# pyannote/pyannote-audio

Hardware: NVIDIA H100
Metric: audio-hours/sec (RTF) community-1 diarization, 16kHz mono, 1/2/4/8 H100 (higher is better)
Workload: dtype f16 tensor-core trunk (f32 accumulate) + split-f16x3 tensor-core segmentation (f32-level accuracy) + f64 clustering

## Files before the change

pyannote_audio_b200/csrc/emb_conv.cu:

```cuda
#include "common.cuh"
#include "emb.cuh"
#include "tc_common.cuh"

namespace b200 {

constexpr int kWgThreads = 288;
constexpr int kTileM = 128;
constexpr int kRowHalo = 8;
constexpr int kMaxSlots = 16;

template <int N, bool WIDE = false, int MH = 1>
__device__ __forceinline__ void conv_epilogue(const float* acc, const ConvParams& p, size_t row, int w0) {
  const int lane = threadIdx.x & 31;
  const int c0 = 2 * (lane & 3) + (WIDE ? (int)blockIdx.y * N : 0);
#pragma unroll
  for (int m = 0; m < MH; ++m)
#pragma unroll
  for (int i = 0; i < 2; ++i) {
    const int w = w0 + 64 * m + ((threadIdx.x >> 5) & 3) * 16 + (lane >> 2) + 8 * i;
    if (w >= p.W_out) continue;
    const size_t pix = (row * p.W_out + w) * (size_t)(WIDE ? p.C_out : N);
    __half2 res[N / 8];
    if (N <= 128 && p.residual) {
#pragma unroll
      for (int j = 0; j < N / 8; ++j) res[j] = *reinterpret_cast<const __half2*>(p.residual + pix + 8 * j + c0);
    }
#pragma unroll
    for (int j = 0; j < N / 8; ++j) {
      const int c = 8 * j + c0;
      const float2 bb = __ldg(reinterpret_cast<const float2*>(p.bias + c));
      float a = acc[m * (N / 2) + 4 * j + 2 * i] + bb.x, d = acc[m * (N / 2) + 4 * j + 2 * i + 1] + bb.y;
      if (p.residual) {
        const float2 r = __half22float2(N <= 128 ? res[j] : *reinterpret_cast<const __half2*>(p.residual + pix + c));
        a += r.x;
        d += r.y;
      }
      if (p.relu) { a = fmaxf(a, 0.f); d = fmaxf(d, 0.f); }
      *reinterpret_cast<__half2*>(p.out + pix + c) = __floats2half2_rn(a, d);
    }
  }
}

template <int N, int CK, bool WIDE = false>
__global__ void __launch_bounds__(kWgThreads, N == 256 ? 1 : 2)
conv_tc_kernel(const __grid_constant__ CUtensorMap tmA, const __grid_constant__ CUtensorMap tmB, ConvParams p) {
  extern __shared__ uint8_t smem_raw[];
  const uint32_t raw = smem_u32(smem_raw);
  const uint32_t base = (raw + 1023u) & ~1023u;
  const uint32_t bar_full = base, bar_empty = base + 64;
  const uint32_t stage0 = base + 1024;
  const uint32_t stage_bytes = p.a_bytes + p.b_bytes;
  const int warp = threadIdx.x >> 5;
  const int wt = blockIdx.x % p.tiles_w;
  const int bh = blockIdx.x / p.tiles_w;
  const int cchunks = p.C_in / CK;

  if (threadIdx.x == 0) {
    for (uint32_t s = 0; s < p.nstages; ++s) { mbar_init(bar_full + 8 * s, 1); mbar_init(bar_empty + 8 * s, 2); }
    asm volatile("fence.mbarrier_init.release.cluster;" ::: "memory");
  }
  __syncthreads();

  if (warp == 8) {
    if ((threadIdx.x & 31) == 0) {
      prefetch_tensormap(&tmA);
      prefetch_tensormap(&tmB);
      const int h = bh % p.H_out, b = bh / p.H_out;
      const int w_base = wt * kTileM * p.stride - p.pad, h_base = h * p.stride - p.pad;
      uint32_t stage = 0, phase = 0;
      for (int kh = 0; kh < p.taps_h; ++kh)
        for (int kw = 0; kw < p.taps_w; ++kw)
          for (int cc = 0; cc < cchunks; ++cc) {
            mbar_wait(bar_empty + 8 * stage, phase ^ 1);
            mbar_expect_tx(bar_full + 8 * stage, p.a_tx + p.b_bytes);
            const uint32_t sa = stage0 + stage * stage_bytes;
            tma_load_4d(&tmA, bar_full + 8 * stage, sa, cc * CK, w_base + kw, h_base + kh, b);
            tma_load_3d(&tmB, bar_full + 8 * stage, sa + p.a_bytes, cc * CK, WIDE ? (int)blockIdx.y * N : 0,
                        kh * p.taps_w + kw);
            if (++stage == p.nstages) { stage = 0; phase ^= 1; }
          }
    }
    return;
  }

  const int wg = warp >> 2;
  constexpr uint32_t row_bytes = CK * 2;
  float acc[N / 2];
#pragma unroll
  for (int i = 0; i < N / 2; ++i) acc[i] = 0.f;
  const int kblocks = p.taps_h * p.taps_w * cchunks;
  uint32_t stage = 0, phase = 0, prev = 0;
  for (int kb = 0; kb < kblocks; ++kb) {
    mbar_wait(bar_full + 8 * stage, phase);
    const uint32_t st = stage0 + stage * stage_bytes;
    const uint32_t sa = st + (uint32_t)wg * 64u * row_bytes, sb = st + p.a_bytes;
    wg_fence();
    const uint64_t ad = wg_desc(sa, row_bytes), bd = wg_desc(sb, row_bytes);
#pragma unroll
    for (int k = 0; k < CK / 16; ++k) Wgmma<N>::mma(acc, ad + 2 * k, bd + 2 * k);
    wg_commit();
    wg_wait<1>();
    if (kb > 0 && (threadIdx.x & 127) == 0) mbar_arrive(bar_empty + 8 * prev);
    prev = stage;
    if (++stage == p.nstages) { stage = 0; phase ^= 1; }
  }
  wg_wait<0>();
  conv_epilogue<N, WIDE>(acc, p, (size_t)bh, wt * kTileM + wg * 64);
}

template <int N>
__device__ __forceinline__ void row_taps_c32(float (&acc)[2][N / 2], uint32_t sa, uint32_t wts) {
  constexpr uint32_t row_bytes = 64;
  const int warp = threadIdx.x >> 5, lane = threadIdx.x & 31;
#pragma unroll
  for (int kw = 0; kw < 3; ++kw) {
    uint32_t af[2][2][4];
#pragma unroll
    for (int m = 0; m < 2; ++m)
#pragma unroll
      for (int k = 0; k < 2; ++k) {
        const uint32_t row = (uint32_t)(m * 64 + (warp & 3) * 16 + (lane & 15) + kw);
        const uint32_t chunk = (uint32_t)(2 * k + (lane >> 4)) ^ ((row >> 1) & 3u);
        ldsm_x4(af[m][k], sa + row * row_bytes + chunk * 16u);
      }
    wg_fence();
    const uint64_t bd = wg_desc(wts + kw * N * row_bytes, row_bytes);
#pragma unroll
    for (int k = 0; k < 2; ++k)
#pragma unroll
      for (int m = 0; m < 2; ++m) WgmmaRS<N>::mma(acc[m], af[m][k], bd + 2 * k);
    wg_commit();
    wg_wait<0>();
  }
}

__device__ __forceinline__ void st_shared_u32(uint32_t a, uint32_t v) {
  asm volatile("st.shared.b32 [%0], %1;" ::"r"(a), "r"(v) : "memory");
}
__device__ __forceinline__ uint32_t ld_shared_u32(uint32_t a) {
  uint32_t v;
  asm volatile("ld.shared.b32 %0, [%1];" : "=r"(v) : "r"(a) : "memory");
  return v;
}
__device__ __forceinline__ uint32_t h2_bits(__half2 h) { return *reinterpret_cast<uint32_t*>(&h); }

template <int N>
struct RowPlan {
  static constexpr uint32_t kRowBytes = N * 2;
  static constexpr uint32_t kTapBytes = N * kRowBytes;
  static constexpr uint32_t kInTx = (kTileM + kRowHalo) * kRowBytes;
  static constexpr uint32_t kSlotBytes = (kInTx + 1023u) & ~1023u;
  static constexpr uint32_t kTileBytes = kTileM * kRowBytes;
  static constexpr uint32_t kSlots = N == 64 ? 7 : 8;
  static constexpr int kResLag = (int)kSlots - 2;
  static constexpr int kCtasPerSm = N == 32 ? 2 : 1;
  static constexpr size_t kBudget = N == 32 ? 113u * 1024 : 227u * 1024;
  static constexpr size_t kSmem = 2048 + 9 * kTapBytes + 2 * kTileBytes + kSlots * kSlotBytes;
  static_assert(N == 32 || N == 64, "row kernel: 32 or 64 channels");
  static_assert(kSlots >= 6 && kSlots <= kMaxSlots, "row ring: four slots in use and two ahead");
  static_assert(kSmem <= kBudget && kSmem + kSlotBytes > kBudget, "row plan: every slot that fits");
};

template <int N, int CK>
__global__ void __launch_bounds__(kWgThreads, N == 32 ? 2 : 1)
conv_row_kernel(const __grid_constant__ CUtensorMap tmA, const __grid_constant__ CUtensorMap tmB,
                const __grid_constant__ CUtensorMap tmR, const __grid_constant__ CUtensorMap tmO, ConvParams p) {
  using P = RowPlan<N>;
  static_assert(CK == N, "row kernel: one channel chunk");
  constexpr uint32_t row_bytes = P::kRowBytes;
  constexpr uint32_t b_tap_bytes = P::kTapBytes;
  constexpr uint32_t nslots = P::kSlots;
  extern __shared__ uint8_t smem_raw[];
  const uint32_t base = (smem_u32(smem_raw) + 1023u) & ~1023u;
  const uint32_t bar_w = base, bar_full = base + 8, bar_empty = base + 8 + 8 * kMaxSlots;
  const uint32_t tile_full = base + 512, tile_empty = base + 528;
  const uint32_t wts = base + 1024;
  const uint32_t tile0 = wts + 9 * b_tap_bytes;
  const uint32_t slot0 = tile0 + 2 * P::kTileBytes;
  const bool has_res = p.residual != nullptr;
  const int warp = threadIdx.x >> 5;

  if (threadIdx.x == 0) {
    mbar_init(bar_w, 1);
    for (uint32_t s = 0; s < nslots; ++s) { mbar_init(bar_full + 8 * s, 1); mbar_init(bar_empty + 8 * s, 3); }
    for (uint32_t s = 0; s < 2; ++s) { mbar_init(tile_full + 8 * s, 1); mbar_init(tile_empty + 8 * s, 1); }
    asm volatile("fence.mbarrier_init.release.cluster;" ::: "memory");
  }
  __syncthreads();

  if (warp == 8) {
    if ((threadIdx.x & 31) == 0) {
      prefetch_tensormap(&tmA);
      prefetch_tensormap(&tmB);
      if (has_res) prefetch_tensormap(&tmR);
      mbar_expect_tx(bar_w, 9 * b_tap_bytes);
      for (int kh = 0; kh < 3; ++kh) tma_load_3d(&tmB, bar_w, wts + 3 * kh * b_tap_bytes, 0, 0, 3 * kh);
      uint32_t s = 0;
      uint32_t k = 0;
      for (int u = blockIdx.x; u < p.num_tiles; u += gridDim.x) {
        const int wt = u % p.tiles_w, t = u / p.tiles_w;
        const int h0 = (t % p.bands) * p.band, b = t / p.bands;
        const int n = min(p.band, p.H_out - h0);
        auto stage_residual = [&](int j) {
          const uint32_t tile = k & 1, use = k >> 1;
          mbar_wait(tile_empty + 8 * tile, (use & 1) ^ 1);
          mbar_expect_tx(tile_full + 8 * tile, P::kTileBytes);
          tma_load_4d(&tmR, tile_full + 8 * tile, tile0 + tile * P::kTileBytes, 0, wt * kTileM, h0 + j, b);
          ++k;
        };
        for (int r = 0; r < n + 2; ++r, ++s) {
          const uint32_t slot = s % nslots;
          mbar_wait(bar_empty + 8 * slot, ((s / nslots) & 1) ^ 1);
          mbar_expect_tx(bar_full + 8 * slot, P::kInTx);
          tma_load_4d(&tmA, bar_full + 8 * slot, slot0 + slot * P::kSlotBytes, 0, wt * kTileM - 1, h0 - 1 + r, b);
          if (has_res && r >= P::kResLag) stage_residual(r - P::kResLag);
        }
        if (has_res)
          for (int j = max(0, n + 2 - P::kResLag); j < n; ++j) stage_residual(j);
      }
    }
    return;
  }

  const int wg = __shfl_sync(0xffffffffu, warp >> 2, 0);
  const int lane = threadIdx.x & 31;
  const bool leader = (threadIdx.x & 127) == 0;
  const uint32_t tile = tile0 + wg * P::kTileBytes;
  const int c0 = 2 * (lane & 3);
  float2 bias[N / 8];
#pragma unroll
  for (int j = 0; j < N / 8; ++j) bias[j] = __ldg(reinterpret_cast<const float2*>(p.bias + 8 * j + c0));
  if (leader) prefetch_tensormap(&tmO);
  mbar_wait(bar_w, 0);
  uint32_t s = 0;
  int item = 0;
  for (int u = blockIdx.x; u < p.num_tiles; u += gridDim.x) {
    const int wt = u % p.tiles_w, t = u / p.tiles_w;
    const int h0 = (t % p.bands) * p.band, b = t / p.bands;
    const int n = min(p.band, p.H_out - h0);
    for (int j = 0; j < n; ++j, ++item) {
      if ((item & 1) != wg) continue;
      float acc[2][N / 2];
#pragma unroll
      for (int m = 0; m < 2; ++m)
#pragma unroll
        for (int i = 0; i < N / 2; ++i) {
          acc[m][i] = 0.f;
          asm volatile("" : "+f"(acc[m][i]));
        }
#pragma unroll
      for (int kh = 0; kh < 3; ++kh) {
        const uint32_t q = s + j + kh, slot = q % nslots;
        mbar_wait(bar_full + 8 * slot, (q / nslots) & 1);
        const uint32_t sa = slot0 + slot * P::kSlotBytes;
        if constexpr (CK == 32) {
          row_taps_c32<N>(acc, sa, wts + 3 * kh * b_tap_bytes);
        } else {
          wg_fence();
#pragma unroll
          for (int kw = 0; kw < 3; ++kw) {
            const uint64_t bd = wg_desc(wts + (3 * kh + kw) * b_tap_bytes, row_bytes);
#pragma unroll
            for (int m = 0; m < 2; ++m) {
              const uint64_t ad = wg_desc(sa + (uint32_t)(m * 64 + kw) * row_bytes, row_bytes);
#pragma unroll
              for (int k = 0; k < CK / 16; ++k) Wgmma<N>::mma(acc[m], ad + 2 * k, bd + 2 * k);
            }
          }
          wg_commit();
        }
      }
      wg_wait<0>();
      if (leader)
#pragma unroll
        for (int kh = 0; kh < 3; ++kh)
          mbar_arrive_n(bar_empty + 8 * ((s + j + kh) % nslots), 1 + (j == 0 ? 2 - kh : 0) + (j == n - 1 ? kh : 0));
      if (has_res) {
        mbar_wait(tile_full + 8 * wg, (item >> 1) & 1);
      } else {
        if (leader) bulk_wait_read<0>();
        named_bar_sync(1 + wg);
      }
#pragma unroll
      for (int m = 0; m < 2; ++m)
#pragma unroll
        for (int i = 0; i < 2; ++i) {
          const uint32_t px = m * 64 + (warp & 3) * 16 + (lane >> 2) + 8 * i;
          const uint32_t swz = row_bytes == 128 ? px & 7u : (px >> 1) & 3u;
#pragma unroll
          for (int jj = 0; jj < N / 8; ++jj) {
            const uint32_t ta = tile + px * row_bytes + ((jj ^ swz) << 4) + 2 * c0;
            float a = acc[m][4 * jj + 2 * i] + bias[jj].x, d = acc[m][4 * jj + 2 * i + 1] + bias[jj].y;
            if (has_res) {
              const uint32_t rb = ld_shared_u32(ta);
              const float2 r = __half22float2(*reinterpret_cast<const __half2*>(&rb));
              a += r.x;
              d += r.y;
            }
            if (p.relu) { a = fmaxf(a, 0.f); d = fmaxf(d, 0.f); }
            st_shared_u32(ta, h2_bits(__floats2half2_rn(a, d)));
          }
        }
      fence_proxy_async();
      named_bar_sync(1 + wg);
      if (leader) {
        tma_store_4d(&tmO, tile, 0, wt * kTileM, h0 + j, b);
        bulk_commit();
        if (has_res) {
          bulk_wait_read<0>();
          mbar_arrive(tile_empty + 8 * wg);
        }
      }
    }
    s += n + 2;
  }
  if (leader) bulk_wait<0>();
}

struct BlockRowPlan {
  static constexpr uint32_t kTapBytes = 32 * 64;
  static constexpr uint32_t kSlotBytes = 9 * 1024;
  static constexpr uint32_t kInTx = (kTileM + kRowHalo) * 64;
  static constexpr uint32_t kInSlots = 4, kMidSlots = 4;
  static constexpr size_t kSmem = 2048 + 2 * 9 * kTapBytes + (kInSlots + kMidSlots) * kSlotBytes;
  static_assert(kInTx <= kSlotBytes && kSmem <= 113 * 1024, "block row plan");
};
constexpr int kStripW = kTileM - 2;

struct BlockParams {
  int H, W, tiles_w, band, bands, num_tiles;
  const float* bias1;
  const float* bias2;
  __half* out;
};


__global__ void __launch_bounds__(kWgThreads, 2)
block_row_kernel(const __grid_constant__ CUtensorMap tmA, const __grid_constant__ CUtensorMap tmW1,
                 const __grid_constant__ CUtensorMap tmW2, BlockParams p) {
  using P = BlockRowPlan;
  constexpr uint32_t NI = P::kInSlots, NM = P::kMidSlots;
  extern __shared__ uint8_t smem_raw[];
  const uint32_t base = (smem_u32(smem_raw) + 1023u) & ~1023u;
  const uint32_t bar_w = base, in_full = base + 8, in_empty = in_full + 8 * NI;
  const uint32_t mid_full = in_empty + 8 * NI, mid_empty = mid_full + 8 * NM;
  const uint32_t w1 = base + 1024, w2 = w1 + 9 * P::kTapBytes;
  const uint32_t in0 = w2 + 9 * P::kTapBytes, mid0 = in0 + NI * P::kSlotBytes;
  const int warp = threadIdx.x >> 5, lane = threadIdx.x & 31;

  if (threadIdx.x == 0) {
    mbar_init(bar_w, 1);
    for (uint32_t s = 0; s < NI; ++s) { mbar_init(in_full + 8 * s, 1); mbar_init(in_empty + 8 * s, 4); }
    for (uint32_t s = 0; s < NM; ++s) { mbar_init(mid_full + 8 * s, 128); mbar_init(mid_empty + 8 * s, 3); }
    asm volatile("fence.mbarrier_init.release.cluster;" ::: "memory");
  }
  __syncthreads();

  if (warp == 8) {
    if (lane == 0) {
      prefetch_tensormap(&tmA);
      prefetch_tensormap(&tmW1);
      prefetch_tensormap(&tmW2);
      mbar_expect_tx(bar_w, 18 * P::kTapBytes);
      for (int kh = 0; kh < 3; ++kh) {
        tma_load_3d(&tmW1, bar_w, w1 + 3 * kh * P::kTapBytes, 0, 0, 3 * kh);
        tma_load_3d(&tmW2, bar_w, w2 + 3 * kh * P::kTapBytes, 0, 0, 3 * kh);
      }
      uint32_t s = 0;
      for (int u = blockIdx.x; u < p.num_tiles; u += gridDim.x) {
        const int wt = u % p.tiles_w, t = u / p.tiles_w;
        const int h0 = (t % p.bands) * p.band, b = t / p.bands;
        const int n = min(p.band, p.H - h0);
        for (int r = 0; r < n + 4; ++r, ++s) {
          const uint32_t slot = s % NI;
          mbar_wait(in_empty + 8 * slot, ((s / NI) & 1) ^ 1);
          mbar_expect_tx(in_full + 8 * slot, P::kInTx);
          tma_load_4d(&tmA, in_full + 8 * slot, in0 + slot * P::kSlotBytes, 0, wt * kStripW - 2, h0 - 2 + r, b);
        }
      }
    }
    return;
  }

  const int wg = __shfl_sync(0xffffffffu, warp >> 2, 0);
  const bool leader = (threadIdx.x & 127) == 0;
  const int c0 = 2 * (lane & 3);
  float2 bias[4];
#pragma unroll
  for (int j = 0; j < 4; ++j) bias[j] = __ldg(reinterpret_cast<const float2*>((wg ? p.bias2 : p.bias1) + 8 * j + c0));
  mbar_wait(bar_w, 0);
  uint32_t s = 0, mq = 0;
  for (int u = blockIdx.x; u < p.num_tiles; u += gridDim.x) {
    const int wt = u % p.tiles_w, t = u / p.tiles_w;
    const int h0 = (t % p.bands) * p.band, b = t / p.bands;
    const int n = min(p.band, p.H - h0);
    const int w0 = wt * kStripW;
    const int rows = wg == 0 ? n + 2 : n;
    for (int j = 0; j < rows; ++j) {
      float acc[2][16];
#pragma unroll
      for (int m = 0; m < 2; ++m)
#pragma unroll
        for (int i = 0; i < 16; ++i) {
          acc[m][i] = 0.f;
          asm volatile("" : "+f"(acc[m][i]));
        }
      if (wg == 0) {
#pragma unroll
        for (int kh = 0; kh < 3; ++kh) {
          const uint32_t q = s + j + kh, slot = q % NI;
          mbar_wait(in_full + 8 * slot, (q / NI) & 1);
          row_taps_c32<32>(acc, in0 + slot * P::kSlotBytes, w1 + 3 * kh * P::kTapBytes);
        }
        if (leader)
#pragma unroll
          for (int kh = 0; kh < 3; ++kh) {
            const int k = j + kh;
            const bool no_res = (k < 2 || k >= n + 2) && j == min(k, n + 1);
            mbar_arrive_n(in_empty + 8 * ((s + k) % NI),
                          1 + (j == 0 ? 2 - kh : 0) + (j == n + 1 ? kh : 0) + (no_res ? 1 : 0));
          }
        const uint32_t q = mq + j, slot = q % NM, sm = mid0 + slot * P::kSlotBytes;
        mbar_wait(mid_empty + 8 * slot, ((q / NM) & 1) ^ 1);
        const int r = h0 - 1 + j;
        const bool live = r >= 0 && r < p.H;
#pragma unroll
        for (int m = 0; m < 2; ++m)
#pragma unroll
          for (int i = 0; i < 2; ++i) {
            const int px = m * 64 + (warp & 3) * 16 + (lane >> 2) + 8 * i, w = w0 - 1 + px;
            const bool in = live && w >= 0 && w < p.W;
#pragma unroll
            for (int jj = 0; jj < 4; ++jj) {
              const float a = fmaxf(acc[m][4 * jj + 2 * i] + bias[jj].x, 0.f);
              const float d = fmaxf(acc[m][4 * jj + 2 * i + 1] + bias[jj].y, 0.f);
              const uint32_t v = in ? h2_bits(__floats2half2_rn(a, d)) : 0u;
              st_shared_u32(sm + px * 64u + ((jj ^ ((px >> 1) & 3)) << 4) + 2 * c0, v);
            }
          }
        mbar_arrive(mid_full + 8 * slot);
      } else {
#pragma unroll
        for (int kh = 0; kh < 3; ++kh) {
          const uint32_t q = mq + j + kh, slot = q % NM;
          mbar_wait(mid_full + 8 * slot, (q / NM) & 1);
          row_taps_c32<32>(acc, mid0 + slot * P::kSlotBytes, w2 + 3 * kh * P::kTapBytes);
        }
        if (leader)
#pragma unroll
          for (int kh = 0; kh < 3; ++kh)
            mbar_arrive_n(mid_empty + 8 * ((mq + j + kh) % NM), 1 + (j == 0 ? 2 - kh : 0) + (j == n - 1 ? kh : 0));
        const uint32_t q = s + j + 2, slot = q % NI, sr = in0 + slot * P::kSlotBytes;
        mbar_wait(in_full + 8 * slot, (q / NI) & 1);
        const size_t row = (size_t)b * p.H + h0 + j;
#pragma unroll
        for (int m = 0; m < 2; ++m)
#pragma unroll
          for (int i = 0; i < 2; ++i) {
            const int px = m * 64 + (warp & 3) * 16 + (lane >> 2) + 8 * i, w = w0 + px;
            if (px >= kStripW || w >= p.W) continue;
            const int rp = px + 2;
            __half2* o = reinterpret_cast<__half2*>(p.out + (row * p.W + w) * 32 + c0);
#pragma unroll
            for (int jj = 0; jj < 4; ++jj) {
              const uint32_t rb = ld_shared_u32(sr + rp * 64u + ((jj ^ ((rp >> 1) & 3)) << 4) + 2 * c0);
              const float2 rv = __half22float2(*reinterpret_cast<const __half2*>(&rb));
              float a = acc[m][4 * jj + 2 * i] + bias[jj].x, d = acc[m][4 * jj + 2 * i + 1] + bias[jj].y;
              a += rv.x;
              d += rv.y;
              o[4 * jj] = __floats2half2_rn(fmaxf(a, 0.f), fmaxf(d, 0.f));
            }
          }
        asm volatile("bar.sync 1, 128;" ::: "memory");
        if (leader) mbar_arrive(in_empty + 8 * slot);
      }
    }
    s += n + 4;
    mq += n + 2;
  }
}

template <int N>
struct ChunkRowPlan {
  static constexpr int kChunks = N / 64;
  static constexpr int kRows = N == 128 ? 2 : 1;
  static constexpr int kHalves = N == 128 ? 2 : 1;
  static constexpr uint32_t kABytes = (kTileM + kRowHalo) * 128;
  static constexpr uint32_t kBBytes = N * 128;
  static constexpr uint32_t kASlots = N == 256 ? 5 : 8;
  static constexpr uint32_t kBSlots = N == 256 ? 4 : 5;
  static constexpr size_t kSmem = 2048 + kASlots * kABytes + kBSlots * kBBytes;
  static_assert(kASlots >= kRows * kChunks + 1 && kASlots <= 8 && kBSlots <= 8, "chunk row ring plan");
  static_assert(kSmem <= 227 * 1024, "chunk row shared memory");
  __device__ __forceinline__ static uint32_t box(int r, int cc) {
    return r < kRows ? cc * kRows + r : kRows * kChunks + (r - kRows) * kChunks + cc;
  }
};

template <int N>
__global__ void __launch_bounds__(kWgThreads, 1)
conv_chunk_row_kernel(const __grid_constant__ CUtensorMap tmA, const __grid_constant__ CUtensorMap tmB, ConvParams p) {
  using P = ChunkRowPlan<N>;
  constexpr int CH = P::kChunks, R = P::kRows, KSTEPS = 9 * CH;
  constexpr uint32_t BOXES = (R + 2) * CH;
  extern __shared__ uint8_t smem_raw[];
  const uint32_t base = (smem_u32(smem_raw) + 1023u) & ~1023u;
  const uint32_t full_a = base, empty_a = base + 64, full_b = base + 128, empty_b = base + 192;
  const uint32_t ring_a = base + 1024, ring_b = ring_a + P::kASlots * P::kABytes;
  const int warp = threadIdx.x >> 5;

  if (threadIdx.x == 0) {
    for (uint32_t s = 0; s < P::kASlots; ++s) { mbar_init(full_a + 8 * s, 1); mbar_init(empty_a + 8 * s, 2); }
    for (uint32_t s = 0; s < P::kBSlots; ++s) { mbar_init(full_b + 8 * s, 1); mbar_init(empty_b + 8 * s, 2); }
    asm volatile("fence.mbarrier_init.release.cluster;" ::: "memory");
  }
  __syncthreads();

  if (warp == 8) {
    if ((threadIdx.x & 31) == 0) {
      prefetch_tensormap(&tmA);
      prefetch_tensormap(&tmB);
      uint32_t qa = 0, qb = 0;
      for (int u = blockIdx.x; u < p.num_tiles; u += gridDim.x) {
        const int wt = u % p.tiles_w, t = u / p.tiles_w;
        const int h = (t % p.bands) * R, b = t / p.bands;
        for (int s = 0; s < KSTEPS; ++s) {
          const int cc = s % CH, kw = (s / CH) % 3, kh = s / (3 * CH);
          if (kw == 0)
            for (int r = kh == 0 ? 0 : kh + R - 1; r < kh + R; ++r) {
              const uint32_t q = qa + P::box(r, cc), slot = q % P::kASlots;
              mbar_wait(empty_a + 8 * slot, ((q / P::kASlots) & 1) ^ 1);
              mbar_expect_tx(full_a + 8 * slot, P::kABytes);
              tma_load_4d(&tmA, full_a + 8 * slot, ring_a + slot * P::kABytes, cc * 64, wt * kTileM - 1, h - 1 + r, b);
            }
          const uint32_t q = qb + s, slot = q % P::kBSlots;
          mbar_wait(empty_b + 8 * slot, ((q / P::kBSlots) & 1) ^ 1);
          mbar_expect_tx(full_b + 8 * slot, P::kBBytes);
          tma_load_3d(&tmB, full_b + 8 * slot, ring_b + slot * P::kBBytes, cc * 64, 0, 3 * kh + kw);
        }
        qa += BOXES;
        qb += KSTEPS;
      }
    }
    return;
  }

  const int wg = __shfl_sync(0xffffffffu, warp >> 2, 0);
  const bool leader = (threadIdx.x & 127) == 0;
  const int ro = R == 2 ? wg : 0;
  uint32_t qa = 0, qb = 0;
  for (int u = blockIdx.x; u < p.num_tiles; u += gridDim.x) {
    const int wt = u % p.tiles_w, t = u / p.tiles_w;
    const int h = (t % p.bands) * R + ro, b = t / p.bands;
    const int w0 = wt * kTileM + (R == 2 ? 0 : wg * 64);
    if (p.residual && h < p.H_out)
#pragma unroll
      for (int l = (threadIdx.x & 127); l < 256; l += 128) {
        const int w = w0 + l / (N / 64);
        if (w < p.W_out)
          asm volatile("prefetch.global.L2 [%0];" ::"l"(p.residual + ((size_t)(b * p.H_out + h) * p.W_out + w) * N +
                                                         (l % (N / 64)) * 64));
      }
    float acc[P::kHalves][N / 2];
#pragma unroll
    for (int m = 0; m < P::kHalves; ++m)
#pragma unroll
      for (int i = 0; i < N / 2; ++i) {
        acc[m][i] = 0.f;
        asm volatile("" : "+f"(acc[m][i]));
      }
    uint32_t prev_b = 0, prev_a = 0, prev_frees_a = 0;
    auto release = [&]() {
      if (leader) {
        mbar_arrive(empty_b + 8 * prev_b);
        if (prev_frees_a) mbar_arrive_n(empty_a + 8 * prev_a, prev_frees_a);
      }
    };
    for (int s = 0; s < KSTEPS; ++s) {
      const int cc = s % CH, kw = (s / CH) % 3, kh = s / (3 * CH);
      const uint32_t qA = qa + P::box(kh + ro, cc), sa = qA % P::kASlots;
      const uint32_t qB = qb + s, sb = qB % P::kBSlots;
      mbar_wait(full_a + 8 * sa, (qA / P::kASlots) & 1);
      mbar_wait(full_b + 8 * sb, (qB / P::kBSlots) & 1);
      wg_fence();
      const uint64_t bd = wg_desc(ring_b + sb * P::kBBytes, 128);
#pragma unroll
      for (int m = 0; m < P::kHalves; ++m) {
        const uint32_t half = R == 2 ? m : wg;
        const uint64_t ad = wg_desc(ring_a + sa * P::kABytes + (half * 64 + kw) * 128u, 128);
#pragma unroll
        for (int k = 0; k < 4; ++k) Wgmma<N>::mma(acc[m], ad + 2 * k, bd + 2 * k);
      }
      wg_commit();
      wg_wait<1>();
      if (s > 0) release();
      prev_b = sb;
      prev_a = sa;
      prev_frees_a = kw == 2 ? (R == 2 && kh == 2 * ro ? 2 : 1) : 0;
    }
    wg_wait<0>();
    release();
    qa += BOXES;
    qb += KSTEPS;
    if (h < p.H_out) conv_epilogue<N, false, P::kHalves>(acc[0], p, (size_t)b * p.H_out + h, w0);
  }
}

__global__ void conv_simt_kernel(const __half* __restrict__ in, const __half* __restrict__ wt, ConvParams p) {
  const int groups = p.C_out / 8;
  const size_t idx = (size_t)blockIdx.x * blockDim.x + threadIdx.x;
  const size_t total = (size_t)p.B * p.H_out * p.W_out * groups;
  if (idx >= total) return;
  const int g = idx % groups;
  size_t pixel = idx / groups;
  const int w = pixel % p.W_out;
  const int h = (pixel / p.W_out) % p.H_out;
  const int b = pixel / ((size_t)p.W_out * p.H_out);
  float acc[8];
#pragma unroll
  for (int j = 0; j < 8; ++j) acc[j] = p.bias[g * 8 + j];
  for (int kh = 0; kh < p.taps_h; ++kh) {
    const int hi = h * p.stride + kh - p.pad;
    if (hi < 0 || hi >= p.H_in) continue;
    for (int kw = 0; kw < p.taps_w; ++kw) {
      const int wi = w * p.stride + kw - p.pad;
      if (wi < 0 || wi >= p.W_in) continue;
      const __half* ip = in + (((size_t)b * p.H_in + hi) * p.W_in + wi) * p.C_in;
      const int tap = kh * p.taps_w + kw;
      for (int ci = 0; ci < p.C_in; ci += 8) {
        uint4 xu = *reinterpret_cast<const uint4*>(ip + ci);
        const __half2* xh = reinterpret_cast<const __half2*>(&xu);
        float x[8];
#pragma unroll
        for (int e = 0; e < 4; ++e) {
          float2 f = __half22float2(xh[e]);
          x[2 * e] = f.x;
          x[2 * e + 1] = f.y;
        }
#pragma unroll
        for (int j = 0; j < 8; ++j) {
          uint4 wu = *reinterpret_cast<const uint4*>(wt + ((size_t)tap * p.C_out + g * 8 + j) * p.C_in + ci);
          const __half2* wh = reinterpret_cast<const __half2*>(&wu);
#pragma unroll
          for (int e = 0; e < 4; ++e) {
            float2 f = __half22float2(wh[e]);
            acc[j] = fmaf(x[2 * e], f.x, acc[j]);
            acc[j] = fmaf(x[2 * e + 1], f.y, acc[j]);
          }
        }
      }
    }
  }
  const size_t o = (((size_t)b * p.H_out + h) * p.W_out + w) * p.C_out + g * 8;
  if (p.residual) {
    uint4 ru = *reinterpret_cast<const uint4*>(p.residual + o);
    const __half2* rh = reinterpret_cast<const __half2*>(&ru);
#pragma unroll
    for (int e = 0; e < 4; ++e) {
      float2 f = __half22float2(rh[e]);
      acc[2 * e] += f.x;
      acc[2 * e + 1] += f.y;
    }
  }
  uint4 ou;
  __half2* oh = reinterpret_cast<__half2*>(&ou);
#pragma unroll
  for (int e = 0; e < 4; ++e) {
    float a = acc[2 * e], c = acc[2 * e + 1];
    if (p.relu) { a = fmaxf(a, 0.f); c = fmaxf(c, 0.f); }
    oh[e] = __floats2half2_rn(a, c);
  }
  *reinterpret_cast<uint4*>(p.out + o) = ou;
}

constexpr int kC1Tile = 128;
__global__ void __launch_bounds__(kC1Tile) conv1_kernel(const float* __restrict__ fbank, const float* __restrict__ fmean,
                             const int* __restrict__ frame0, const float* __restrict__ w , const float* __restrict__ bias ,
                             __half* __restrict__ out, int T0) {
  __shared__ __align__(16) float sw[9 * 32];
  __shared__ __align__(16) float sb[32];
  __shared__ float sx[(kC1Tile + 2) * (kMel + 1)];
  const int b = blockIdx.x, t0 = blockIdx.y * kC1Tile;
  const size_t r0 = frame0 ? (size_t)frame0[b] : (size_t)b * T0;
  for (int i = threadIdx.x; i < 288; i += blockDim.x) sw[(i % 9) * 32 + i / 9] = w[i];
  if (threadIdx.x < 32) sb[threadIdx.x] = bias[threadIdx.x];
  for (int i = threadIdx.x; i < (kC1Tile + 2) * kMel; i += blockDim.x) {
    const int tt = i / kMel, f = i - tt * kMel;
    const int t = t0 - 1 + tt;
    float v = 0.f;
    if (t >= 0 && t < T0) v = fbank[(r0 + t) * kMel + f] - fmean[(size_t)b * kMel + f];
    sx[tt * (kMel + 1) + f] = v;
  }
  __syncthreads();
  const int t = t0 + threadIdx.x;
  if (t >= T0) return;
  const float* col = sx + threadIdx.x * (kMel + 1);
  for (int h = 0; h < kMel; ++h) {
    asm volatile("" ::: "memory");
    float x[9];
#pragma unroll
    for (int kh = 0; kh < 3; ++kh) {
      const int hh = h + kh - 1;
      const bool ok = hh >= 0 && hh < kMel;
#pragma unroll
      for (int kw = 0; kw < 3; ++kw) x[kh * 3 + kw] = ok ? col[kw * (kMel + 1) + hh] : 0.f;
    }
    f32x2_t acc2[16];
    const ulonglong2* sb2 = reinterpret_cast<const ulonglong2*>(sb);
#pragma unroll
    for (int q = 0; q < 8; ++q) { const ulonglong2 bb = sb2[q]; acc2[2 * q] = bb.x; acc2[2 * q + 1] = bb.y; }
#pragma unroll
    for (int k = 0; k < 9; ++k) {
      const f32x2_t xk = pack2(x[k], x[k]);
      const ulonglong2* wk = reinterpret_cast<const ulonglong2*>(sw + k * 32);
#pragma unroll
      for (int q = 0; q < 8; ++q) {
        const ulonglong2 w4 = wk[q];
        ffma2(acc2[2 * q], xk, w4.x);
        ffma2(acc2[2 * q + 1], xk, w4.y);
      }
    }
    __half2 o[16];
#pragma unroll
    for (int c = 0; c < 16; ++c) {
      float a0, a1;
      unpack2(acc2[c], a0, a1);
      o[c] = __floats2half2_rn(fmaxf(a0, 0.f), fmaxf(a1, 0.f));
    }
    uint4* op = reinterpret_cast<uint4*>(out + (((size_t)b * kMel + h) * T0 + t) * 32);
    const uint4* src = reinterpret_cast<const uint4*>(o);
#pragma unroll
    for (int i = 0; i < 4; ++i) op[i] = src[i];
  }
}

typedef CUresult (*PFN_encodeTiled)(CUtensorMap*, CUtensorMapDataType, cuuint32_t, void*, const cuuint64_t*,
                                    const cuuint64_t*, const cuuint32_t*, const cuuint32_t*, CUtensorMapInterleave,
                                    CUtensorMapSwizzle, CUtensorMapL2promotion, CUtensorMapFloatOOBfill);

static PFN_encodeTiled get_encode() {
  static PFN_encodeTiled fn = nullptr;
  if (!fn) {
    void* ptr = nullptr;
    cudaDriverEntryPointQueryResult qres;
    if (cudaGetDriverEntryPoint("cuTensorMapEncodeTiled", &ptr, cudaEnableDefault, &qres) == cudaSuccess &&
        qres == cudaDriverEntryPointSuccess)
      fn = reinterpret_cast<PFN_encodeTiled>(ptr);
  }
  return fn;
}

int encode_f16_map(CUtensorMap* tm, int rank, const void* ptr, const cuuint64_t* dims, const cuuint64_t* strides,
                   const cuuint32_t* box, const cuuint32_t* estr, CUtensorMapSwizzle swizzle, const char* what) {
  PFN_encodeTiled enc = get_encode();
  B200_CHECK(enc != nullptr, B200_ERR_CUDA, "cuTensorMapEncodeTiled not available from the driver");
  const cuuint32_t ones[5] = {1, 1, 1, 1, 1};
  CUresult r = enc(tm, CU_TENSOR_MAP_DATA_TYPE_FLOAT16, (cuuint32_t)rank, const_cast<void*>(ptr), dims, strides, box,
                   estr ? estr : ones, CU_TENSOR_MAP_INTERLEAVE_NONE, swizzle, CU_TENSOR_MAP_L2_PROMOTION_L2_256B,
                   CU_TENSOR_MAP_FLOAT_OOB_FILL_NONE);
  B200_CHECK(r == CUDA_SUCCESS, B200_ERR_CUDA, "cuTensorMapEncodeTiled(%s) failed: %d", what, (int)r);
  return B200_OK;
}

int conv_forward(const ConvLayer& L, const __half* in, const __half* residual, __half* out, int B, int H_in, int W_in,
                 int relu, int impl, int num_sms, cudaStream_t stream) {
  ConvParams p{};
  p.B = B; p.H_in = H_in; p.W_in = W_in; p.C_in = L.C_in; p.C_out = L.C_out;
  p.taps_h = L.ksize; p.taps_w = L.ksize; p.stride = L.stride; p.pad = L.ksize / 2;
  p.H_out = (H_in + 2 * p.pad - L.ksize) / L.stride + 1;
  p.W_out = (W_in + 2 * p.pad - L.ksize) / L.stride + 1;
  p.relu = relu; p.bias = L.bias; p.residual = residual; p.out = out;
  p.Ck = (L.C_in >= 64) ? 64 : 32;
  p.swizzle = (p.Ck == 64) ? 128 : 64;
  p.tiles_w = ceil_div(p.W_out, kTileM);
  p.num_tiles = B * p.H_out * p.tiles_w;
  B200_CHECK(L.C_in % p.Ck == 0 && (L.C_out == 32 || L.C_out == 64 || L.C_out == 128 ||
                                    (L.C_out % 256 == 0 && L.C_out <= 1024 && p.Ck == 64)),
             B200_ERR_STATE, "conv %d -> %d channels unsupported", L.C_in, L.C_out);
  const int n_tile = std::min(L.C_out, 256);
  B200_CHECK(impl >= 0 && impl <= 2, B200_ERR_INVALID,
             "conv_impl %d unknown (0 = CUDA cores, 1 = tensor cores, 2 = tensor cores, one weight tap per stage)", impl);

  if (impl == 0) {
    const size_t total = (size_t)B * p.H_out * p.W_out * (L.C_out / 8);
    return launch(conv_simt_kernel, (unsigned)((total + 255) / 256), 256, 0, stream, in, L.w, p);
  }

  const bool rows = impl == 1 && L.ksize == 3 && L.stride == 1 && L.C_in == p.Ck && L.C_out == L.C_in;
  const bool chunk_rows =
      impl == 1 && L.ksize == 3 && L.stride == 1 && L.C_out == L.C_in && (L.C_out == 128 || L.C_out == 256);
  p.a_rows = rows || chunk_rows ? kTileM + kRowHalo : kTileM;
  p.a_tx = p.a_rows * p.Ck * 2;
  p.a_bytes = (p.a_tx + 1023u) & ~1023u;
  size_t smem;
  int ctas = 0;
  if (rows) {
    const int per_sm = L.C_out == 32 ? RowPlan<32>::kCtasPerSm : RowPlan<64>::kCtasPerSm;
    smem = L.C_out == 32 ? RowPlan<32>::kSmem : RowPlan<64>::kSmem;
    ctas = per_sm * num_sms;
    const int strips = B * p.tiles_w;
    const int nbands = std::min(p.H_out, ceil_div(ctas, strips));
    p.band = ceil_div(p.H_out, nbands);
    p.bands = ceil_div(p.H_out, p.band);
    p.num_tiles = strips * p.bands;
  } else if (chunk_rows) {
    p.band = L.C_out == 256 ? ChunkRowPlan<256>::kRows : ChunkRowPlan<128>::kRows;
    p.bands = ceil_div(p.H_out, p.band);
    p.num_tiles = B * p.bands * p.tiles_w;
    smem = L.C_out == 256 ? ChunkRowPlan<256>::kSmem : ChunkRowPlan<128>::kSmem;
    ctas = num_sms;
  } else {
    p.b_bytes = (uint32_t)(n_tile * p.Ck * 2);
    const uint32_t budget = n_tile == 256 ? 200u * 1024 : 100u * 1024;
    p.nstages = std::min(budget / (p.a_bytes + p.b_bytes), 8u);
    B200_CHECK(p.nstages >= 2, B200_ERR_STATE, "conv %d -> %d: shared memory plan too shallow", L.C_in, L.C_out);
    smem = 1024 + 1024 + (size_t)p.nstages * (p.a_bytes + p.b_bytes);
  }
  const CUtensorMapSwizzle swz = p.swizzle == 128 ? CU_TENSOR_MAP_SWIZZLE_128B : CU_TENSOR_MAP_SWIZZLE_64B;
  CUtensorMap tmA, tmB;
  int rc;
  {
    const cuuint64_t dims[4] = {(cuuint64_t)L.C_in, (cuuint64_t)W_in, (cuuint64_t)H_in, (cuuint64_t)B};
    const cuuint64_t strides[3] = {(cuuint64_t)L.C_in * 2, (cuuint64_t)W_in * L.C_in * 2,
                                   (cuuint64_t)H_in * W_in * L.C_in * 2};
    const cuuint32_t box[4] = {(cuuint32_t)p.Ck, (cuuint32_t)(p.a_rows * L.stride), 1, 1};
    const cuuint32_t estr[4] = {1, (cuuint32_t)L.stride, 1, 1};
    if ((rc = encode_f16_map(&tmA, 4, in, dims, strides, box, estr, swz, "A"))) return rc;
  }
  {
    const cuuint64_t dims[3] = {(cuuint64_t)L.C_in, (cuuint64_t)L.C_out, (cuuint64_t)(L.ksize * L.ksize)};
    const cuuint64_t strides[2] = {(cuuint64_t)L.C_in * 2, (cuuint64_t)L.C_out * L.C_in * 2};
    const cuuint32_t box[3] = {(cuuint32_t)p.Ck, (cuuint32_t)n_tile, rows ? 3u : 1u};
    if ((rc = encode_f16_map(&tmB, 3, L.w, dims, strides, box, nullptr, swz, "B"))) return rc;
  }
  if (rows) {
    CUtensorMap tmR{}, tmO;
    const cuuint64_t dims[4] = {(cuuint64_t)L.C_out, (cuuint64_t)p.W_out, (cuuint64_t)p.H_out, (cuuint64_t)B};
    const cuuint64_t strides[3] = {(cuuint64_t)L.C_out * 2, (cuuint64_t)p.W_out * L.C_out * 2,
                                   (cuuint64_t)p.H_out * p.W_out * L.C_out * 2};
    const cuuint32_t box[4] = {(cuuint32_t)L.C_out, (cuuint32_t)kTileM, 1, 1};
    if (residual && (rc = encode_f16_map(&tmR, 4, residual, dims, strides, box, nullptr, swz, "residual"))) return rc;
    if ((rc = encode_f16_map(&tmO, 4, out, dims, strides, box, nullptr, swz, "out"))) return rc;
    auto kernel = p.Ck == 32 ? conv_row_kernel<32, 32> : conv_row_kernel<64, 64>;
    return launch(kernel, (unsigned)std::min(p.num_tiles, ctas), kWgThreads, smem, stream, tmA, tmB, tmR, tmO, p);
  }
  const dim3 grid((unsigned)(ctas ? std::min(p.num_tiles, ctas) : p.num_tiles), (unsigned)(L.C_out / n_tile));
  auto run = [&](auto kernel) { return launch(kernel, grid, kWgThreads, smem, stream, tmA, tmB, p); };
  if (chunk_rows) return L.C_out == 256 ? run(conv_chunk_row_kernel<256>) : run(conv_chunk_row_kernel<128>);
  if (p.Ck == 32) {
    switch (L.C_out) {
      case 32: return run(conv_tc_kernel<32, 32>);
      case 64: return run(conv_tc_kernel<64, 32>);
      default: return run(conv_tc_kernel<128, 32>);
    }
  }
  switch (L.C_out) {
    case 32: return run(conv_tc_kernel<32, 64>);
    case 64: return run(conv_tc_kernel<64, 64>);
    case 128: return run(conv_tc_kernel<128, 64>);
    case 256: return run(conv_tc_kernel<256, 64>);
    default: return run(conv_tc_kernel<256, 64, true>);
  }
}

bool block_fused(const BlockWeights& Bw, int impl) {
  return impl == 1 && !Bw.has_shortcut && Bw.conv1.stride == 1 && Bw.conv1.ksize == 3 && Bw.conv2.ksize == 3 &&
         Bw.conv1.C_in == 32 && Bw.conv1.C_out == 32 && Bw.conv2.C_in == 32 && Bw.conv2.C_out == 32;
}

int block_forward(const BlockWeights& Bw, const __half* in, __half* out, int B, int H, int W, int num_sms,
                  cudaStream_t stream) {
  B200_CHECK(block_fused(Bw, 1), B200_ERR_STATE, "block %d -> %d (stride %d) has no fused kernel", Bw.conv1.C_in,
             Bw.conv1.C_out, Bw.conv1.stride);
  B200_CHECK(in != out, B200_ERR_INVALID, "fused block: output must not alias the input");
  BlockParams p{};
  p.H = H; p.W = W; p.bias1 = Bw.conv1.bias; p.bias2 = Bw.conv2.bias; p.out = out;
  p.tiles_w = ceil_div(W, kStripW);
  const int ctas = 2 * num_sms;
  const int strips = B * p.tiles_w;
  const int nbands = std::min(H, ceil_div(ctas, strips));
  p.band = ceil_div(H, nbands);
  p.bands = ceil_div(H, p.band);
  p.num_tiles = strips * p.bands;
  CUtensorMap tmA, tmW1, tmW2;
  int rc;
  {
    const cuuint64_t dims[4] = {32, (cuuint64_t)W, (cuuint64_t)H, (cuuint64_t)B};
    const cuuint64_t strides[3] = {64, (cuuint64_t)W * 64, (cuuint64_t)H * W * 64};
    const cuuint32_t box[4] = {32, kTileM + kRowHalo, 1, 1};
    if ((rc = encode_f16_map(&tmA, 4, in, dims, strides, box, nullptr, CU_TENSOR_MAP_SWIZZLE_64B, "block A"))) return rc;
  }
  {
    const cuuint64_t dims[3] = {32, 32, 9};
    const cuuint64_t strides[2] = {64, 32 * 64};
    const cuuint32_t box[3] = {32, 32, 3};
    if ((rc = encode_f16_map(&tmW1, 3, Bw.conv1.w, dims, strides, box, nullptr, CU_TENSOR_MAP_SWIZZLE_64B, "block W1")))
      return rc;
    if ((rc = encode_f16_map(&tmW2, 3, Bw.conv2.w, dims, strides, box, nullptr, CU_TENSOR_MAP_SWIZZLE_64B, "block W2")))
      return rc;
  }
  const size_t smem = BlockRowPlan::kSmem;
  return launch(block_row_kernel, (unsigned)std::min(p.num_tiles, ctas), kWgThreads, smem, stream, tmA, tmW1, tmW2, p);
}

int conv1_forward(const float* fbank, const float* fmean, const int* frame0, const float* w, const float* bias,
                  __half* out, int B, int T0, cudaStream_t stream) {
  dim3 grid(B, ceil_div(T0, kC1Tile));
  return launch(conv1_kernel, grid, kC1Tile, 0, stream, fbank, fmean, frame0, w, bias, out, T0);
}

}
```

Baseline: 1.968.

## Add row-streaming TMA kernel for stride-2 ResNet convolutions

Adds a persistent row-band kernel for stride-2 convolutions (3x3 32->64 and 1x1 shortcuts 32->64, 64->128). A producer warp streams input rows through a ring of TMA-loaded slots, with even and odd column phases loaded separately, so each loaded input row serves the overlapping 3x3 taps of adjacent output rows instead of being reloaded per tap. The epilogue is factored into a shared helper that supports two 128-B swizzled output boxes. The change adds more shared-memory ring logic and barrier counting, and runs one CTA per SM.

```diff
diff --git a/pyannote_audio_b200/csrc/emb_conv.cu b/pyannote_audio_b200/csrc/emb_conv.cu
--- a/pyannote_audio_b200/csrc/emb_conv.cu
+++ b/pyannote_audio_b200/csrc/emb_conv.cu
@@ -108,20 +108,22 @@
   conv_epilogue<N, WIDE>(acc, p, (size_t)bh, wt * kTileM + wg * 64);
 }
 
-template <int N>
-__device__ __forceinline__ void row_taps_c32(float (&acc)[2][N / 2], uint32_t sa, uint32_t wts) {
+template <int N, int S = 1>
+__device__ __forceinline__ void row_taps_c32(float (&acc)[2][N / 2], uint32_t sa, uint32_t wts, uint32_t odd = 0) {
   constexpr uint32_t row_bytes = 64;
   const int warp = threadIdx.x >> 5, lane = threadIdx.x & 31;
 #pragma unroll
   for (int kw = 0; kw < 3; ++kw) {
+    const uint32_t box = S == 1 || kw == 1 ? sa : odd;
+    const int shift = S == 1 ? kw : kw / 2;
     uint32_t af[2][2][4];
 #pragma unroll
     for (int m = 0; m < 2; ++m)
 #pragma unroll
       for (int k = 0; k < 2; ++k) {
-        const uint32_t row = (uint32_t)(m * 64 + (warp & 3) * 16 + (lane & 15) + kw);
+        const uint32_t row = (uint32_t)(m * 64 + (warp & 3) * 16 + (lane & 15) + shift);
         const uint32_t chunk = (uint32_t)(2 * k + (lane >> 4)) ^ ((row >> 1) & 3u);
-        ldsm_x4(af[m][k], sa + row * row_bytes + chunk * 16u);
+        ldsm_x4(af[m][k], box + row * row_bytes + chunk * 16u);
       }
     wg_fence();
     const uint64_t bd = wg_desc(wts + kw * N * row_bytes, row_bytes);
@@ -143,6 +145,33 @@
   return v;
 }
 __device__ __forceinline__ uint32_t h2_bits(__half2 h) { return *reinterpret_cast<uint32_t*>(&h); }
+
+template <int N>
+__device__ __forceinline__ void row_tile_epilogue(const float (&acc)[2][N / 2], const float2 (&bias)[N / 8],
+                                                  uint32_t tile, bool has_res, const ConvParams& p, int warp,
+                                                  int lane, int c0) {
+  constexpr uint32_t row_bytes = N > 64 ? 128 : N * 2;
+#pragma unroll
+  for (int m = 0; m < 2; ++m)
+#pragma unroll
+    for (int i = 0; i < 2; ++i) {
+      const uint32_t px = m * 64 + (warp & 3) * 16 + (lane >> 2) + 8 * i;
+      const uint32_t swz = row_bytes == 128 ? px & 7u : (px >> 1) & 3u;
+#pragma unroll
+      for (int jj = 0; jj < N / 8; ++jj) {
+        const uint32_t ta = tile + (jj / 8) * (kTileM * 128) + px * row_bytes + (((jj % 8) ^ swz) << 4) + 2 * c0;
+        float a = acc[m][4 * jj + 2 * i] + bias[jj].x, d = acc[m][4 * jj + 2 * i + 1] + bias[jj].y;
+        if (has_res) {
+          const uint32_t rb = ld_shared_u32(ta);
+          const float2 r = __half22float2(*reinterpret_cast<const __half2*>(&rb));
+          a += r.x;
+          d += r.y;
+        }
+        if (p.relu) { a = fmaxf(a, 0.f); d = fmaxf(d, 0.f); }
+        st_shared_u32(ta, h2_bits(__floats2half2_rn(a, d)));
+      }
+    }
+}
 
 template <int N>
 struct RowPlan {
@@ -281,26 +310,7 @@
         if (leader) bulk_wait_read<0>();
         named_bar_sync(1 + wg);
       }
-#pragma unroll
-      for (int m = 0; m < 2; ++m)
-#pragma unroll
-        for (int i = 0; i < 2; ++i) {
-          const uint32_t px = m * 64 + (warp & 3) * 16 + (lane >> 2) + 8 * i;
-          const uint32_t swz = row_bytes == 128 ? px & 7u : (px >> 1) & 3u;
-#pragma unroll
-          for (int jj = 0; jj < N / 8; ++jj) {
-            const uint32_t ta = tile + px * row_bytes + ((jj ^ swz) << 4) + 2 * c0;
-            float a = acc[m][4 * jj + 2 * i] + bias[jj].x, d = acc[m][4 * jj + 2 * i + 1] + bias[jj].y;
-            if (has_res) {
-              const uint32_t rb = ld_shared_u32(ta);
-              const float2 r = __half22float2(*reinterpret_cast<const __half2*>(&rb));
-              a += r.x;
-              d += r.y;
-            }
-            if (p.relu) { a = fmaxf(a, 0.f); d = fmaxf(d, 0.f); }
-            st_shared_u32(ta, h2_bits(__floats2half2_rn(a, d)));
-          }
-        }
+      row_tile_epilogue<N>(acc, bias, tile, has_res, p, warp, lane, c0);
       fence_proxy_async();
       named_bar_sync(1 + wg);
       if (leader) {
@@ -313,6 +323,149 @@
       }
     }
     s += n + 2;
+  }
+  if (leader) bulk_wait<0>();
+}
+
+template <int N, int CK, int KS>
+struct S2RowPlan {
+  static constexpr uint32_t kInRowBytes = CK * 2;
+  static constexpr uint32_t kTapBytes = N * kInRowBytes;
+  static constexpr uint32_t kMainTx = kTileM * kInRowBytes;
+  static constexpr uint32_t kPhaseBytes = ((kTileM + kRowHalo) * kInRowBytes + 1023u) & ~1023u;
+  static constexpr int kPhases = KS == 3 ? 2 : 1;
+  static constexpr uint32_t kSlotBytes = kPhases * kPhaseBytes;
+  static constexpr uint32_t kInTx = KS == 3 ? 2 * kMainTx + kRowHalo * kInRowBytes : kMainTx;
+  static constexpr uint32_t kTileBytes = kTileM * N * 2;
+  static constexpr size_t kFixed = 2048 + KS * KS * kTapBytes + 2 * kTileBytes;
+  static constexpr uint32_t kSlots = std::min<size_t>(kMaxSlots, (227u * 1024 - kFixed) / kSlotBytes);
+  static constexpr size_t kSmem = kFixed + kSlots * kSlotBytes;
+  static_assert(N == 64 || N == 128, "s2 row kernel: the output row is one or two 128-B swizzled TMA boxes");
+  static_assert(KS == 1 || CK == 32, "s2 row kernel: the 3x3 taps read 64-B rows through row_taps_c32");
+  static_assert(kSlots >= 2 * KS, "s2 row ring: the rows of two output rows and one ahead");
+};
+
+template <int N, int CK, int KS>
+__global__ void __launch_bounds__(kWgThreads, 1)
+conv_s2_row_kernel(const __grid_constant__ CUtensorMap tmA, const __grid_constant__ CUtensorMap tmT,
+                   const __grid_constant__ CUtensorMap tmB, const __grid_constant__ CUtensorMap tmO, ConvParams p) {
+  using P = S2RowPlan<N, CK, KS>;
+  constexpr uint32_t nslots = P::kSlots;
+  extern __shared__ uint8_t smem_raw[];
+  const uint32_t base = (smem_u32(smem_raw) + 1023u) & ~1023u;
+  const uint32_t bar_w = base, bar_full = base + 8, bar_empty = base + 8 + 8 * kMaxSlots;
+  const uint32_t wts = base + 1024;
+  const uint32_t tile0 = wts + KS * KS * P::kTapBytes;
+  const uint32_t slot0 = tile0 + 2 * P::kTileBytes;
+  const int warp = threadIdx.x >> 5;
+
+  if (threadIdx.x == 0) {
+    mbar_init(bar_w, 1);
+    for (uint32_t s = 0; s < nslots; ++s) { mbar_init(bar_full + 8 * s, 1); mbar_init(bar_empty + 8 * s, 2); }
+    asm volatile("fence.mbarrier_init.release.cluster;" ::: "memory");
+  }
+  __syncthreads();
+
+  if (warp == 8) {
+    if ((threadIdx.x & 31) == 0) {
+      prefetch_tensormap(&tmA);
+      if (KS == 3) prefetch_tensormap(&tmT);
+      prefetch_tensormap(&tmB);
+      mbar_expect_tx(bar_w, KS * KS * P::kTapBytes);
+      for (int kh = 0; kh < KS; ++kh) tma_load_3d(&tmB, bar_w, wts + KS * kh * P::kTapBytes, 0, 0, KS * kh);
+      uint32_t s = 0;
+      for (int u = blockIdx.x; u < p.num_tiles; u += gridDim.x) {
+        const int wt = u % p.tiles_w, t = u / p.tiles_w;
+        const int h0 = (t % p.bands) * p.band, b = t / p.bands;
+        const int n = min(p.band, p.H_out - h0);
+        const int x = 2 * wt * kTileM;
+        for (int r = 0; r < (KS == 3 ? 2 * n + 1 : n); ++r, ++s) {
+          const uint32_t slot = s % nslots, dst = slot0 + slot * P::kSlotBytes, full = bar_full + 8 * slot;
+          const int hi = KS == 3 ? 2 * h0 - 1 + r : 2 * (h0 + r);
+          mbar_wait(bar_empty + 8 * slot, ((s / nslots) & 1) ^ 1);
+          mbar_expect_tx(full, P::kInTx);
+          tma_load_4d(&tmA, full, dst, 0, x, hi, b);
+          if (KS == 3) {
+            tma_load_4d(&tmA, full, dst + P::kPhaseBytes, 0, x - 1, hi, b);
+            tma_load_4d(&tmT, full, dst + P::kPhaseBytes + P::kMainTx, 0, x - 1 + 2 * kTileM, hi, b);
+          }
+        }
+      }
+    }
+    return;
+  }
+
+  const int wg = __shfl_sync(0xffffffffu, warp >> 2, 0);
+  const int lane = threadIdx.x & 31;
+  const bool leader = (threadIdx.x & 127) == 0;
+  const uint32_t tile = tile0 + wg * P::kTileBytes;
+  const int c0 = 2 * (lane & 3);
+  float2 bias[N / 8];
+#pragma unroll
+  for (int j = 0; j < N / 8; ++j) bias[j] = __ldg(reinterpret_cast<const float2*>(p.bias + 8 * j + c0));
+  if (leader) prefetch_tensormap(&tmO);
+  mbar_wait(bar_w, 0);
+  uint32_t s = 0;
+  int item = 0;
+  for (int u = blockIdx.x; u < p.num_tiles; u += gridDim.x) {
+    const int wt = u % p.tiles_w, t = u / p.tiles_w;
+    const int h0 = (t % p.bands) * p.band, b = t / p.bands;
+    const int n = min(p.band, p.H_out - h0);
+    for (int j = 0; j < n; ++j, ++item) {
+      if ((item & 1) != wg) continue;
+      float acc[2][N / 2];
+#pragma unroll
+      for (int m = 0; m < 2; ++m)
+#pragma unroll
+        for (int i = 0; i < N / 2; ++i) {
+          acc[m][i] = 0.f;
+          asm volatile("" : "+f"(acc[m][i]));
+        }
+      if constexpr (KS == 3) {
+#pragma unroll
+        for (int kh = 0; kh < 3; ++kh) {
+          const uint32_t q = s + 2 * j + kh, slot = q % nslots;
+          mbar_wait(bar_full + 8 * slot, (q / nslots) & 1);
+          const uint32_t sa = slot0 + slot * P::kSlotBytes;
+          row_taps_c32<N, 2>(acc, sa, wts + 3 * kh * P::kTapBytes, sa + P::kPhaseBytes);
+        }
+      } else {
+        const uint32_t q = s + j, slot = q % nslots;
+        mbar_wait(bar_full + 8 * slot, (q / nslots) & 1);
+        const uint32_t sa = slot0 + slot * P::kSlotBytes;
+        wg_fence();
+        const uint64_t bd = wg_desc(wts, P::kInRowBytes);
+#pragma unroll
+        for (int m = 0; m < 2; ++m) {
+          const uint64_t ad = wg_desc(sa + (uint32_t)m * 64u * P::kInRowBytes, P::kInRowBytes);
+#pragma unroll
+          for (int k = 0; k < CK / 16; ++k) Wgmma<N>::mma(acc[m], ad + 2 * k, bd + 2 * k);
+        }
+        wg_commit();
+      }
+      wg_wait<0>();
+      if (leader) {
+        if constexpr (KS == 3) {
+#pragma unroll
+          for (int kh = 0; kh < 3; ++kh)
+            mbar_arrive_n(bar_empty + 8 * ((s + 2 * j + kh) % nslots),
+                          kh == 1 || (kh == 0 && j == 0) || (kh == 2 && j == n - 1) ? 2 : 1);
+        } else {
+          mbar_arrive_n(bar_empty + 8 * ((s + j) % nslots), 2);
+        }
+        bulk_wait_read<0>();
+      }
+      named_bar_sync(1 + wg);
+      row_tile_epilogue<N>(acc, bias, tile, false, p, warp, lane, c0);
+      fence_proxy_async();
+      named_bar_sync(1 + wg);
+      if (leader) {
+#pragma unroll
+        for (int c = 0; c < N; c += 64) tma_store_4d(&tmO, tile + c / 64 * (kTileM * 128), c, wt * kTileM, h0 + j, b);
+        bulk_commit();
+      }
+    }
+    s += KS == 3 ? 2 * n + 1 : n;
   }
   if (leader) bulk_wait<0>();
 }
@@ -789,14 +942,20 @@
   const bool rows = impl == 1 && L.ksize == 3 && L.stride == 1 && L.C_in == p.Ck && L.C_out == L.C_in;
   const bool chunk_rows =
       impl == 1 && L.ksize == 3 && L.stride == 1 && L.C_out == L.C_in && (L.C_out == 128 || L.C_out == 256);
+  const bool s2_rows = impl == 1 && L.stride == 2 &&
+                       ((L.C_in == 32 && L.C_out == 64) || (L.ksize == 1 && L.C_in == 64 && L.C_out == 128));
   p.a_rows = rows || chunk_rows ? kTileM + kRowHalo : kTileM;
   p.a_tx = p.a_rows * p.Ck * 2;
   p.a_bytes = (p.a_tx + 1023u) & ~1023u;
   size_t smem;
   int ctas = 0;
-  if (rows) {
-    const int per_sm = L.C_out == 32 ? RowPlan<32>::kCtasPerSm : RowPlan<64>::kCtasPerSm;
-    smem = L.C_out == 32 ? RowPlan<32>::kSmem : RowPlan<64>::kSmem;
+  if (rows || s2_rows) {
+    const int per_sm = s2_rows ? 1 : L.C_out == 32 ? RowPlan<32>::kCtasPerSm : RowPlan<64>::kCtasPerSm;
+    if (s2_rows)
+      smem = L.ksize == 3 ? S2RowPlan<64, 32, 3>::kSmem
+                          : L.C_out == 64 ? S2RowPlan<64, 32, 1>::kSmem : S2RowPlan<128, 64, 1>::kSmem;
+    else
+      smem = L.C_out == 32 ? RowPlan<32>::kSmem : RowPlan<64>::kSmem;
     ctas = per_sm * num_sms;
     const int strips = B * p.tiles_w;
     const int nbands = std::min(p.H_out, ceil_div(ctas, strips));
@@ -830,17 +989,31 @@
   {
     const cuuint64_t dims[3] = {(cuuint64_t)L.C_in, (cuuint64_t)L.C_out, (cuuint64_t)(L.ksize * L.ksize)};
     const cuuint64_t strides[2] = {(cuuint64_t)L.C_in * 2, (cuuint64_t)L.C_out * L.C_in * 2};
-    const cuuint32_t box[3] = {(cuuint32_t)p.Ck, (cuuint32_t)n_tile, rows ? 3u : 1u};
+    const cuuint32_t box[3] = {(cuuint32_t)p.Ck, (cuuint32_t)n_tile, (rows || s2_rows) && L.ksize == 3 ? 3u : 1u};
     if ((rc = encode_f16_map(&tmB, 3, L.w, dims, strides, box, nullptr, swz, "B"))) return rc;
   }
-  if (rows) {
+  if (rows || s2_rows) {
     CUtensorMap tmR{}, tmO;
     const cuuint64_t dims[4] = {(cuuint64_t)L.C_out, (cuuint64_t)p.W_out, (cuuint64_t)p.H_out, (cuuint64_t)B};
     const cuuint64_t strides[3] = {(cuuint64_t)L.C_out * 2, (cuuint64_t)p.W_out * L.C_out * 2,
                                    (cuuint64_t)p.H_out * p.W_out * L.C_out * 2};
-    const cuuint32_t box[4] = {(cuuint32_t)L.C_out, (cuuint32_t)kTileM, 1, 1};
-    if (residual && (rc = encode_f16_map(&tmR, 4, residual, dims, strides, box, nullptr, swz, "residual"))) return rc;
-    if ((rc = encode_f16_map(&tmO, 4, out, dims, strides, box, nullptr, swz, "out"))) return rc;
+    const cuuint32_t box[4] = {(cuuint32_t)std::min(L.C_out, 64), (cuuint32_t)kTileM, 1, 1};
+    const CUtensorMapSwizzle swz_out = L.C_out >= 64 ? CU_TENSOR_MAP_SWIZZLE_128B : CU_TENSOR_MAP_SWIZZLE_64B;
+    if (residual && (rc = encode_f16_map(&tmR, 4, residual, dims, strides, box, nullptr, swz_out, "residual")))
+      return rc;
+    if ((rc = encode_f16_map(&tmO, 4, out, dims, strides, box, nullptr, swz_out, "out"))) return rc;
+    if (s2_rows) {
+      CUtensorMap tmT{};
+      const cuuint64_t dims[4] = {(cuuint64_t)L.C_in, (cuuint64_t)W_in, (cuuint64_t)H_in, (cuuint64_t)B};
+      const cuuint64_t strides[3] = {(cuuint64_t)L.C_in * 2, (cuuint64_t)W_in * L.C_in * 2,
+                                     (cuuint64_t)H_in * W_in * L.C_in * 2};
+      const cuuint32_t box[4] = {(cuuint32_t)p.Ck, 2 * kRowHalo, 1, 1};
+      const cuuint32_t estr[4] = {1, 2, 1, 1};
+      if (L.ksize == 3 && (rc = encode_f16_map(&tmT, 4, in, dims, strides, box, estr, swz, "A tail"))) return rc;
+      auto kernel = L.ksize == 3 ? conv_s2_row_kernel<64, 32, 3>
+                    : L.C_out == 64 ? conv_s2_row_kernel<64, 32, 1> : conv_s2_row_kernel<128, 64, 1>;
+      return launch(kernel, (unsigned)std::min(p.num_tiles, ctas), kWgThreads, smem, stream, tmA, tmT, tmB, tmO, p);
+    }
     auto kernel = p.Ck == 32 ? conv_row_kernel<32, 32> : conv_row_kernel<64, 64>;
     return launch(kernel, (unsigned)std::min(p.num_tiles, ctas), kWgThreads, smem, stream, tmA, tmB, tmR, tmO, p);
   }
```

Result: faster. 2.008 (median of 6 runs) (+2.0%).
